# IN2-ViAUn/Exploration-of-Potential

Measured on AMD Instinct MI355X. Metric: training images/sec, YOLOX-l 24p 640x640 bf16, higher is better.
Workload: dtype bf16; 1 GPU; YOLOX-l-24p (CSPDarknet53+PAFPN+24p head) train step, 640x640, batch 20/GPU, 10 GTs/img, SimOTA + 24-circle GIoU loss, SGD nesterov; global_batch=20, parallelism=dp1, hip_graph=forward and backward as two lanes of captured segments, loss, update

## Files before the change

### exploration-of-potential_amd/csrc/elementwise.hip

```cpp
#include <stdio.h>
#include <stdlib.h>
#include "common.h"

namespace {

constexpr int MAX_BLOCKS = 2048;

__device__ __forceinline__ void load8(const bf16* p, float (&v)[8]) {
    bf16x8 t = *reinterpret_cast<const bf16x8*>(p);
#pragma unroll
    for (int i = 0; i < 8; ++i) v[i] = (float)t[i];
}
__device__ __forceinline__ void store8(bf16* p, const float (&v)[8]) {
    bf16x8 t;
#pragma unroll
    for (int i = 0; i < 8; ++i) t[i] = (bf16)v[i];
    *reinterpret_cast<bf16x8*>(p) = t;
}

struct RowMap {
    int tpr, rpb;
    __device__ RowMap(int C, int nt = 256) { tpr = C >> 3; rpb = tpr >= nt ? 1 : nt / tpr; }
};

template <int ACT, bool RES>
__global__ __launch_bounds__(256) void bn_act_fwd_kernel(const bf16* z, long ld_z, const long long* stats, int reps,
                                                         const float* gamma, const float* beta, float* rmean,
                                                         float* rvar, long* nbt, long* nbt2, float* save, bf16* y, long ld_y,
                                                         const bf16* res_, long ld_res, long M, int C, float eps,
                                                         float momentum) {
    constexpr int act = ACT;
    const bf16* res = RES ? res_ : nullptr;
    extern __shared__ float lds[];
    const int CP = C + (C >> 3);
    float* sc = lds;
    float* sh = lds + CP;
    auto pad = [](int c) { return c + (c >> 3); };
    for (int c = threadIdx.x; c < C; c += 256) {
        long long i1 = 0, i2 = 0;
        const float gmm = gamma[c], bta = beta[c];
        for (int rb = 0; rb < reps; rb += 8) {
            long long a[8], b[8];
#pragma unroll
            for (int r = 0; r < 8; ++r) {
                const int rr = rb + r < reps ? rb + r : rb;
                a[r] = stats[(long)rr * 2 * C + c];
                b[r] = stats[(long)rr * 2 * C + C + c];
            }
#pragma unroll
            for (int r = 0; r < 8; ++r) {
                i1 += rb + r < reps ? a[r] : 0ll;
                i2 += rb + r < reps ? b[r] : 0ll;
            }
        }
        const float mean = from_fix(i1) / (float)M;
        float var = from_fix(i2) / (float)M - mean * mean;
        var = var < 0.f ? 0.f : var;
        const float invstd = rsqrtf(var + eps);
        const float s_ = gmm * invstd;
        sc[pad(c)] = s_;
        sh[pad(c)] = bta - mean * s_;
        if (blockIdx.x == 0) {
            save[c] = mean;
            save[C + c] = invstd;
            if (rmean) {
                const float unb = M > 1 ? var * (float)M / (float)(M - 1) : var;
                rmean[c] = (1.f - momentum) * rmean[c] + momentum * mean;
                rvar[c] = (1.f - momentum) * rvar[c] + momentum * unb;
            }
        }
    }
    if (blockIdx.x == 0 && threadIdx.x == 0) {
        if (nbt) *nbt += 1;
        if (nbt2) *nbt2 += 1;
    }
    __syncthreads();
    const int cgs = C >> 3;
    const long total = M * cgs;
    const long stride = (long)gridDim.x * 256;
    constexpr int U = 4;
    const bool fixed_group = stride % cgs == 0;
    const int g_fixed = (int)(((long)blockIdx.x * 256 + threadIdx.x) % cgs);
    float rsc[8], rsh[8];
#pragma unroll
    for (int j = 0; j < 8; ++j) { rsc[j] = sc[g_fixed * 9 + j]; rsh[j] = sh[g_fixed * 9 + j]; }
    const long m_fixed = ((long)blockIdx.x * 256 + threadIdx.x) / cgs, m_step = stride / cgs;
    int it = 0;
    for (long i = (long)blockIdx.x * 256 + threadIdx.x; i < total; i += U * stride, ++it) {
        long mm[U];
        int gg[U];
        bf16x8 v[U], r[U];
#pragma unroll
        for (int k = 0; k < U; ++k) {
            const long ik = i + k * stride;
            const bool ok = ik < total;
            if (fixed_group) {
                mm[k] = ok ? m_fixed + (long)(it * U + k) * m_step : -1;
                gg[k] = g_fixed;
            } else {
                mm[k] = ok ? ik / cgs : -1;
                gg[k] = ok ? (int)(ik - mm[k] * cgs) : 0;
            }
            if (ok) {
                v[k] = *reinterpret_cast<const bf16x8*>(z + mm[k] * ld_z + gg[k] * 8);
                if constexpr (RES) r[k] = *reinterpret_cast<const bf16x8*>(res + mm[k] * ld_res + gg[k] * 8);
            }
        }
#pragma unroll
        for (int k = 0; k < U; ++k) {
            if (mm[k] < 0) break;
            bf16x8 o;
#pragma unroll
            for (int j = 0; j < 8; ++j) {
                const float a_ = fixed_group ? rsc[j] : sc[gg[k] * 9 + j];
                const float b_ = fixed_group ? rsh[j] : sh[gg[k] * 9 + j];
                const float u = fmaf((float)v[k][j], a_, b_);
                if constexpr (RES) o[j] = (bf16)(act_fwd(u, act) + (float)r[k][j]);
                else o[j] = (bf16)act_fwd(u, act);
            }
            *reinterpret_cast<bf16x8*>(y + mm[k] * ld_y + gg[k] * 8) = o;
        }
    }
}


template <int UNROLL, int NT, int ACT>
__device__ __forceinline__ void bn_bwd_reduce_body(const bf16* dy, long ld_dy, const bf16* z, long ld_z,
                                                   const float* save, const float* gamma,
                                                   const float* beta, long long* dgamma, long long* dbeta,
                                                   long M, int C, int reps, const int bid, const int nblk) {
    constexpr int act = ACT;
    __shared__ float red[NT][8 + 1];
    const RowMap rm(C, NT);
    const int tid = threadIdx.x;
    for (int cg0 = 0; cg0 < (C >> 3); cg0 += NT) {
        const int cg = cg0 + tid % rm.tpr;
        const int slot = rm.tpr >= NT ? 0 : tid / rm.tpr;
        const bool active = slot < rm.rpb && cg < (C >> 3);
        float sg[8] = {0, 0, 0, 0, 0, 0, 0, 0}, sb[8] = {0, 0, 0, 0, 0, 0, 0, 0};
        if (active) {
            const long step = (long)nblk * rm.rpb;
            const long m_first = (long)bid * rm.rpb + slot;
            bf16x8 vdy[UNROLL], vz[UNROLL];
#pragma unroll
            for (int k = 0; k < UNROLL; ++k) {
                const long mm = m_first + k * step < M ? m_first + k * step : (m_first < M ? m_first : 0);
                vdy[k] = *reinterpret_cast<const bf16x8*>(dy + mm * ld_dy + cg * 8);
                vz[k] = *reinterpret_cast<const bf16x8*>(z + mm * ld_z + cg * 8);
            }
            __builtin_amdgcn_sched_barrier(0);
            float sc[8], sh[8], iv[8], mi[8];
#pragma unroll
            for (int j = 0; j < 8; ++j) {
                const int c = cg * 8 + j;
                const float mean = save[c], inv = save[C + c];
                sc[j] = gamma[c] * inv; sh[j] = beta[c] - mean * sc[j]; iv[j] = inv; mi[j] = mean * inv;
            }
            for (long m = m_first; m < M; m += UNROLL * step) {
#pragma unroll
                for (int k = 0; k < UNROLL; ++k) {
                    if (m + k * step >= M) break;
#pragma unroll
                    for (int j = 0; j < 8; ++j) {
                        const float zz = (float)vz[k][j];
                        const float du = (float)vdy[k][j] * act_grad(fmaf(zz, sc[j], sh[j]), act);
                        sb[j] += du;
                        sg[j] = fmaf(du, fmaf(zz, iv[j], -mi[j]), sg[j]);
                    }
                }
                if (m + UNROLL * step < M) {
#pragma unroll
                    for (int k = 0; k < UNROLL; ++k) {
                        const long mn = m + (UNROLL + k) * step;
                        const long mm = mn < M ? mn : m;
                        vdy[k] = *reinterpret_cast<const bf16x8*>(dy + mm * ld_dy + cg * 8);
                        vz[k] = *reinterpret_cast<const bf16x8*>(z + mm * ld_z + cg * 8);
                    }
                }
            }
        }
        const int ngrp = min(min(rm.tpr, NT), (C >> 3) - cg0);
#pragma unroll
        for (int half = 0; half < 2; ++half) {
#pragma unroll
            for (int j = 0; j < 8; ++j) red[tid][j] = half ? sb[j] : sg[j];
            __syncthreads();
            for (int t = tid; t < ngrp * 8; t += NT) {
                const int g = t >> 3, v = t & 7;
                float a = 0.f;
                for (int sl = 0; sl < rm.rpb; ++sl) a += red[sl * rm.tpr + g][v];
                long long* dst = (half ? dbeta : dgamma) + (long)(bid % reps) * 2 * C + (cg0 + g) * 8 + v;
                atomicAdd((unsigned long long*)dst, (unsigned long long)to_fix_g(a));
            }
            __syncthreads();
        }
    }
}

template <int UNROLL, int NT, int ACT>
__global__ __launch_bounds__(NT) void bn_act_bwd_reduce_kernel(const bf16* dy, long ld_dy, const bf16* z, long ld_z,
                                                               const float* save, const float* gamma,
                                                               const float* beta, long long* dgamma, long long* dbeta,
                                                               long M, int C, int reps) {
    bn_bwd_reduce_body<UNROLL, NT, ACT>(dy, ld_dy, z, ld_z, save, gamma, beta, dgamma, dbeta, M, C, reps, (int)blockIdx.x, (int)gridDim.x);
}

template <int UNROLL, int ACT, bool ACC, bool COH>
__device__ __forceinline__ void bn_bwd_apply_body(const bf16* dy, long ld_dy, const bf16* z, long ld_z,
                                                  const float* save, const float* gamma, const float* beta,
                                                  const long long* dgamma, const long long* dbeta, float* ggrad,
                                                  float* bgrad, bf16* dz, long ld_dz, long M, int C, int reps, const int bid, const int nblk) {
    constexpr int act = ACT;
    const RowMap rm(C);
    const int tid = threadIdx.x;
    const float invM = 1.f / (float)M;
    extern __shared__ float folded[];
    for (int i = tid; i < 2 * C; i += 256) {
        const long long* src = i < C ? dgamma + i : dbeta + (i - C);
        long long acc = 0;
        bool bad = false;
        for (int rb = 0; rb < reps; rb += 8) {
            long long a[8];
#pragma unroll
            for (int r = 0; r < 8; ++r) {
                const long long* q = src + (long)(rb + r < reps ? rb + r : rb) * 2 * C;
                a[r] = COH ? __hip_atomic_load(q, __ATOMIC_RELAXED, __HIP_MEMORY_SCOPE_AGENT) : *q;
            }
#pragma unroll
            for (int r = 0; r < 8; ++r) {
                acc += rb + r < reps ? a[r] : 0ll;
                bad = bad || fixg_bad(a[r]);
            }
        }
        folded[i] = bad ? __builtin_nanf("") : from_fix_g(acc);
    }
    __syncthreads();
    for (int cg = tid % rm.tpr; cg < (C >> 3); cg += 256) {
        const int slot = rm.tpr >= 256 ? 0 : tid / rm.tpr;
        if (slot >= rm.rpb) break;
        float sc[8], sh[8], k1[8], k2[8], k3[8];
        float cm[8], ci[8], cg_[8], cb[8], csg[8], csb[8];
        {
            const f32x4* pm = reinterpret_cast<const f32x4*>(save + cg * 8);
            const f32x4* pi = reinterpret_cast<const f32x4*>(save + C + cg * 8);
            const f32x4* pg = reinterpret_cast<const f32x4*>(gamma + cg * 8);
            const f32x4* pb = reinterpret_cast<const f32x4*>(beta + cg * 8);
            const f32x4 m0 = pm[0], m1 = pm[1], i0 = pi[0], i1 = pi[1], g0 = pg[0], g1 = pg[1], b0 = pb[0], b1 = pb[1];
            const f32x4 s0 = *reinterpret_cast<const f32x4*>(folded + cg * 8), s1 = *reinterpret_cast<const f32x4*>(folded + cg * 8 + 4);
            const f32x4 t0 = *reinterpret_cast<const f32x4*>(folded + C + cg * 8), t1 = *reinterpret_cast<const f32x4*>(folded + C + cg * 8 + 4);
#pragma unroll
            for (int j = 0; j < 4; ++j) {
                cm[j] = m0[j]; cm[4 + j] = m1[j]; ci[j] = i0[j]; ci[4 + j] = i1[j]; cg_[j] = g0[j]; cg_[4 + j] = g1[j]; cb[j] = b0[j]; cb[4 + j] = b1[j];
                csg[j] = s0[j]; csg[4 + j] = s1[j]; csb[j] = t0[j]; csb[4 + j] = t1[j];
            }
        }
#pragma unroll
        for (int j = 0; j < 8; ++j) {
            const float mean = cm[j], inv = ci[j], g = cg_[j];
            const float sg_ = csg[j], sb_ = csb[j];
            sc[j] = g * inv; sh[j] = cb[j] - mean * sc[j];
            k1[j] = g * inv;
            k3[j] = k1[j] * inv * (sg_ * invM);
            k2[j] = k1[j] * (sb_ * invM) - k3[j] * mean;
        }
        if (bid == 0 && slot == 0 && ggrad) {
            f32x4* pgg = reinterpret_cast<f32x4*>(ggrad + cg * 8);
            f32x4* pbg = reinterpret_cast<f32x4*>(bgrad + cg * 8);
            f32x4 a0 = pgg[0], a1 = pgg[1], c0 = pbg[0], c1 = pbg[1];
#pragma unroll
            for (int j = 0; j < 4; ++j) {
                a0[j] += csg[j]; a1[j] += csg[4 + j];
                c0[j] += csb[j]; c1[j] += csb[4 + j];
            }
            pgg[0] = a0; pgg[1] = a1; pbg[0] = c0; pbg[1] = c1;
        }
        const long step = (long)nblk * rm.rpb;
        for (long m = (long)bid * rm.rpb + slot; m < M; m += UNROLL * step) {
            bf16x8 vdy[UNROLL], vz[UNROLL];
#pragma unroll
            for (int k = 0; k < UNROLL; ++k) {
                const long mm = m + k * step;
                if (mm < M) {
                    vdy[k] = __builtin_nontemporal_load(reinterpret_cast<const bf16x8*>(dy + mm * ld_dy + cg * 8));
                    vz[k] = __builtin_nontemporal_load(reinterpret_cast<const bf16x8*>(z + mm * ld_z + cg * 8));
                }
            }
#pragma unroll
            for (int k = 0; k < UNROLL; ++k) {
                const long mm = m + k * step;
                if (mm >= M) break;
                bf16x8 o;
#pragma unroll
                for (int j = 0; j < 8; ++j) {
                    const float zz = (float)vz[k][j];
                    const float du = (float)vdy[k][j] * act_grad(fmaf(zz, sc[j], sh[j]), act);
                    o[j] = (bf16)fmaf(-k3[j], zz, fmaf(k1[j], du, -k2[j]));
                }
                if (ACC) {
                    const bf16x8 old = *reinterpret_cast<const bf16x8*>(dz + mm * ld_dz + cg * 8);
#pragma unroll
                    for (int j = 0; j < 8; ++j) o[j] = (bf16)((float)old[j] + (float)o[j]);
                }
                *reinterpret_cast<bf16x8*>(dz + mm * ld_dz + cg * 8) = o;
            }
        }
    }
}

template <int UNROLL, int ACT, bool ACC = false>
__global__ __launch_bounds__(256) void bn_act_bwd_apply_kernel(const bf16* dy, long ld_dy, const bf16* z, long ld_z,
                                                               const float* save, const float* gamma, const float* beta,
                                                               const long long* dgamma, const long long* dbeta, float* ggrad,
                                                               float* bgrad, bf16* dz, long ld_dz, long M, int C, int reps) {
    bn_bwd_apply_body<UNROLL, ACT, ACC, false>(dy, ld_dy, z, ld_z, save, gamma, beta, dgamma, dbeta, ggrad, bgrad, dz, ld_dz, M, C, reps,
                                               (int)blockIdx.x, (int)gridDim.x);
}

__device__ unsigned g_bn_barrier_timeouts;

template <int ACT>
__global__ __launch_bounds__(256) void bn_act_bwd_fused_kernel(const bf16* dy, long ld_dy, const bf16* z, long ld_z,
                                                               const float* save, const float* gamma, const float* beta,
                                                               long long* dgamma, long long* dbeta, float* ggrad, float* bgrad,
                                                               bf16* dz, long ld_dz, long M, int C, int reps, unsigned* bar) {
    const int bid = (int)blockIdx.x, nblk = (int)gridDim.x;
    bn_bwd_reduce_body<4, 256, ACT>(dy, ld_dy, z, ld_z, save, gamma, beta, dgamma, dbeta, M, C, reps, bid, nblk);
    __syncthreads();
    if (threadIdx.x == 0) {
        __threadfence();
        __hip_atomic_fetch_add(bar, 1u, __ATOMIC_RELEASE, __HIP_MEMORY_SCOPE_AGENT);
        int tries = 0;
        while (__hip_atomic_load(bar, __ATOMIC_ACQUIRE, __HIP_MEMORY_SCOPE_AGENT) < (unsigned)nblk) {
            __builtin_amdgcn_s_sleep(2);
            if (++tries > (1 << 16)) { atomicAdd(&g_bn_barrier_timeouts, 1u); break; }
        }
    }
    __syncthreads();
    bn_bwd_apply_body<4, ACT, false, true>(dy, ld_dy, z, ld_z, save, gamma, beta, dgamma, dbeta, ggrad, bgrad, dz, ld_dz, M, C, reps, bid, nblk);
}

int flat_grid(long M, int C, int per_thread) {
    long blocks = (M * (C >> 3) + 256L * per_thread - 1) / (256L * per_thread);
    return (int)(blocks < 1 ? 1 : (blocks > MAX_BLOCKS ? MAX_BLOCKS : blocks));
}
int rows_grid(long M, int C, int rows_per_thread, int max_blocks, int nt = 256) {
    int tpr = C >> 3;
    int rpb = tpr >= nt ? 1 : nt / tpr;
    long blocks = (M + (long)rpb * rows_per_thread - 1) / ((long)rpb * rows_per_thread);
    return (int)(blocks < 1 ? 1 : (blocks > max_blocks ? max_blocks : blocks));
}

__global__ __launch_bounds__(256) void stem_pack_kernel(const float* img, bf16* rows, int B, int IH, int IW, int ld) {
    constexpr int TP = 32;
    __shared__ __attribute__((aligned(16))) bf16 tile[TP][120];
    const int FH = IH >> 1, FW = IW >> 1;
    const long npix = (long)B * FH * FW;
    const int chunks = ld >> 3;
    for (long p0 = (long)blockIdx.x * TP; p0 < npix; p0 += (long)gridDim.x * TP) {
        for (int it = threadIdx.x; it < 9 * TP; it += 256) {
            const int tap = it / TP, lp = it - tap * TP;
            const long pix = p0 + lp;
            float v[12] = {0.f, 0.f, 0.f, 0.f, 0.f, 0.f, 0.f, 0.f, 0.f, 0.f, 0.f, 0.f};
            if (pix < npix) {
                const int n = (int)(pix / ((long)FH * FW));
                const int rem = (int)(pix - (long)n * FH * FW);
                const int oy = rem / FW, ox = rem - oy * FW;
                const int fy = oy + tap / 3 - 1, fx = ox + tap % 3 - 1;
                if (fy >= 0 && fy < FH && fx >= 0 && fx < FW) {
#pragma unroll
                    for (int ch = 0; ch < 3; ++ch)
#pragma unroll
                        for (int yp = 0; yp < 2; ++yp) {
                            const float2 t = *reinterpret_cast<const float2*>(img + (((long)n * 3 + ch) * IH + 2 * fy + yp) * IW + 2 * fx);
                            v[(0 * 2 + yp) * 3 + ch] = t.x;
                            v[(1 * 2 + yp) * 3 + ch] = t.y;
                        }
                }
            }
#pragma unroll
            for (int j = 0; j < 12; ++j) tile[lp][tap * 12 + j] = (bf16)v[j];
        }
        if (threadIdx.x < TP) {
#pragma unroll
            for (int j = 108; j < 120; ++j) tile[threadIdx.x][j] = (bf16)0.f;
        }
        __syncthreads();
        for (int it = threadIdx.x; it < TP * chunks; it += 256) {
            const int lp = it / chunks, c = it - lp * chunks;
            const long pix = p0 + lp;
            if (pix >= npix) continue;
            bf16x8 o = {0, 0, 0, 0, 0, 0, 0, 0};
            if (c * 8 < 120) o = *reinterpret_cast<const bf16x8*>(&tile[lp][c * 8]);
            *reinterpret_cast<bf16x8*>(rows + pix * ld + c * 8) = o;
        }
        __syncthreads();
    }
}

__global__ __launch_bounds__(256) void focus_pack_kernel(const float* img, bf16* out, int B, int IH, int IW) {
    const int FH = IH >> 1, FW = IW >> 1;
    const long npix = (long)B * FH * FW;
    for (long pix = (long)blockIdx.x * 256 + threadIdx.x; pix < npix; pix += (long)gridDim.x * 256) {
        const int n = (int)(pix / ((long)FH * FW));
        const int rem = (int)(pix - (long)n * FH * FW);
        const int fy = rem / FW, fx = rem - fy * FW;
        float v[12];
#pragma unroll
        for (int ch = 0; ch < 3; ++ch)
#pragma unroll
            for (int yp = 0; yp < 2; ++yp) {
                const float2 t = *reinterpret_cast<const float2*>(img + (((long)n * 3 + ch) * IH + 2 * fy + yp) * IW + 2 * fx);
                v[(0 * 2 + yp) * 3 + ch] = t.x;
                v[(1 * 2 + yp) * 3 + ch] = t.y;
            }
        bf16x8 lo, hi = {0, 0, 0, 0, 0, 0, 0, 0};
#pragma unroll
        for (int j = 0; j < 8; ++j) lo[j] = (bf16)v[j];
#pragma unroll
        for (int j = 8; j < 12; ++j) hi[j - 8] = (bf16)v[j];
        *reinterpret_cast<bf16x8*>(out + pix * 16) = lo;
        *reinterpret_cast<bf16x8*>(out + pix * 16 + 8) = hi;
    }
}

__global__ __launch_bounds__(256) void spp_fwd_kernel(const bf16* x, long ld_x, bf16* y5, bf16* y9, bf16* y13, long ld_y,
                                                      uint8_t* idx, int B, int H, int W, int C) {
    const int cgs = C >> 3;
    const long total = (long)B * H * W * cgs;
    const long plane = (long)B * H * W * C;
    for (long i = (long)blockIdx.x * 256 + threadIdx.x; i < total; i += (long)gridDim.x * 256) {
        const int cg = (int)(i % cgs);
        const long pix = i / cgs;
        const int n = (int)(pix / (H * W));
        const int rem = (int)(pix - (long)n * H * W);
        const int py = rem / W, px = rem - py * W;
        float m5[8], m9[8], m13[8];
        uint8_t i5[8], i9[8], i13[8];
#pragma unroll
        for (int j = 0; j < 8; ++j) { m5[j] = m9[j] = m13[j] = -INFINITY; i5[j] = i9[j] = i13[j] = 0x88; }
        for (int dy = -6; dy <= 6; ++dy) {
            const int yy = py + dy;
            if (yy < 0 || yy >= H) continue;
            for (int dx = -6; dx <= 6; ++dx) {
                const int xx = px + dx;
                if (xx < 0 || xx >= W) continue;
                float v[8];
                load8(x + ((long)(n * H + yy) * W + xx) * ld_x + cg * 8, v);
                const uint8_t code = (uint8_t)(((dy + 8) << 4) | (dx + 8));
                const bool in9 = dy >= -4 && dy <= 4 && dx >= -4 && dx <= 4;
                const bool in5 = dy >= -2 && dy <= 2 && dx >= -2 && dx <= 2;
#pragma unroll
                for (int j = 0; j < 8; ++j) {
                    if (v[j] > m13[j] || v[j] != v[j]) { m13[j] = v[j]; i13[j] = code; }
                    if (in9 && (v[j] > m9[j] || v[j] != v[j])) { m9[j] = v[j]; i9[j] = code; }
                    if (in5 && (v[j] > m5[j] || v[j] != v[j])) { m5[j] = v[j]; i5[j] = code; }
                }
            }
        }
        store8(y5 + pix * ld_y + cg * 8, m5);
        store8(y9 + pix * ld_y + cg * 8, m9);
        store8(y13 + pix * ld_y + cg * 8, m13);
        uint8_t* ip = idx + pix * C + cg * 8;
#pragma unroll
        for (int j = 0; j < 8; ++j) { ip[j] = i5[j]; ip[plane + j] = i9[j]; ip[2 * plane + j] = i13[j]; }
    }
}

__global__ __launch_bounds__(256) void spp_row_kernel(const bf16* x, long ld_x, bf16* h, uint8_t* hx, int B, int H, int W, int C) {
    const int cgs = C >> 3;
    const long total = (long)B * H * W * cgs;
    const long plane = (long)B * H * W * C;
    for (long i = (long)blockIdx.x * 256 + threadIdx.x; i < total; i += (long)gridDim.x * 256) {
        const int cg = (int)(i % cgs);
        const long pix = i / cgs;
// ... 541 lines not shown
constexpr int WF_NONE = -2147483647 - 1;
__global__ __launch_bounds__(256) void sgd_kernel(float* p, const float* g, float* buf, long n, float lr, float mom,
                                                  float gscale, const int* first_flag, const float* hp, float* ema,
                                                  long base = 0, const int* wf_delta = nullptr, bf16* wf = nullptr) {
    const int first = *first_flag;
    float d = 0.f, omd = 0.f;
    if (hp) { lr = hp[0]; mom = hp[1]; gscale = hp[2]; d = hp[3]; omd = hp[4]; }
    for (long i = ((long)blockIdx.x * 256 + threadIdx.x) * 4; i < n; i += (long)gridDim.x * 1024) {
        if (i + 3 < n) {
            f32x4 gv = *reinterpret_cast<const f32x4*>(g + i);
            f32x4 pv = *reinterpret_cast<const f32x4*>(p + i);
            f32x4 bv = first ? (f32x4){0.f, 0.f, 0.f, 0.f} : *reinterpret_cast<const f32x4*>(buf + i);
            const int wd = wf_delta ? wf_delta[(base + i) >> 6] : WF_NONE;
#pragma unroll
            for (int j = 0; j < 4; ++j) {
                const float gg = gv[j] * gscale;
                bv[j] = first ? gg : mom * bv[j] + gg;
                pv[j] -= lr * (gg + mom * bv[j]);
            }
            *reinterpret_cast<f32x4*>(buf + i) = bv;
            *reinterpret_cast<f32x4*>(p + i) = pv;
            if (wd != WF_NONE) {
                bf16x4 o;
#pragma unroll
                for (int j = 0; j < 4; ++j) o[j] = (bf16)pv[j];
                *reinterpret_cast<bf16x4*>(wf + (base + i + wd)) = o;
            }
            if (ema) {
                f32x4 ev = *reinterpret_cast<const f32x4*>(ema + i);
#pragma unroll
                for (int j = 0; j < 4; ++j) ev[j] = ema_step(ev[j], pv[j], d, omd);
                *reinterpret_cast<f32x4*>(ema + i) = ev;
            }
        } else {
            for (long k = i; k < n; ++k) {
                const float gg = g[k] * gscale;
                const float b = first ? gg : mom * buf[k] + gg;
                buf[k] = b;
                p[k] -= lr * (gg + mom * b);
                if (ema) ema[k] = ema_step(ema[k], p[k], d, omd);
                const int wd = wf_delta ? wf_delta[(base + k) >> 6] : WF_NONE;
                if (wd != WF_NONE) wf[base + k + wd] = (bf16)p[k];
            }
        }
    }
}

__global__ __launch_bounds__(256) void ema_kernel(float* ema, const float* src, long n, float d, float omd, const float* hp) {
    if (hp) { d = hp[3]; omd = hp[4]; }
    for (long i = (long)blockIdx.x * 256 + threadIdx.x; i < n; i += (long)gridDim.x * 256) ema[i] = ema_step(ema[i], src[i], d, omd);
}

__global__ void set_hparams_kernel(float* hp, float lr, float mom, float gscale, float d, float omd) {
    hp[0] = lr; hp[1] = mom; hp[2] = gscale; hp[3] = d; hp[4] = omd;
}
__global__ void clear_flag_kernel(int* f) { *f = 0; }

int cap_grid(long work_items) {
    long b = (work_items + 255) / 256;
    return (int)(b < 1 ? 1 : (b > MAX_BLOCKS ? MAX_BLOCKS : b));
}

}

#define S_ (hipStream_t) stream

extern "C" int ep24_bn_act_fwd(const void* z, int64_t ld_z, const int64_t* stats, int reps, const float* gamma,
                               const float* beta, float* running_mean, float* running_var, int64_t* num_batches,
                               int64_t* num_batches2, float* save, void* y, int64_t ld_y, const void* residual, int64_t ld_res,
                               int64_t M, int C, float eps, float momentum, int act, void* stream) {
    EP24_REQUIRE(act >= 0 && act <= 3, EP24_E_ARG, "bn_act_fwd: act=%d is none of 0 identity, 1 SiLU, 2 ReLU, 3 LeakyReLU(0.1)", act);
    EP24_REQUIRE(z && stats && gamma && beta && save && y, EP24_E_ARG, "bn_act_fwd: null pointer");
    EP24_REQUIRE(C % 8 == 0 && ld_z % 8 == 0 && ld_y % 8 == 0 && (!residual || ld_res % 8 == 0), EP24_E_ARG,
                 "bn_act_fwd: C=%d / strides must be multiples of 8", C);
    EP24_REQUIRE(M > 0 && reps > 0, EP24_E_ARG, "bn_act_fwd: empty");
    const int fw_per = (C >= 1024 || (C <= 128 && M * C >= (12L << 20))) ? 8 : 4;
    auto kfn = residual ? (act == 1 ? bn_act_fwd_kernel<1, true> : act == 2 ? bn_act_fwd_kernel<2, true> : act == 3 ? bn_act_fwd_kernel<3, true> : bn_act_fwd_kernel<0, true>)
                        : (act == 1 ? bn_act_fwd_kernel<1, false> : act == 2 ? bn_act_fwd_kernel<2, false> : act == 3 ? bn_act_fwd_kernel<3, false> : bn_act_fwd_kernel<0, false>);
    hipLaunchKernelGGL(kfn, dim3(flat_grid(M, C, fw_per)), dim3(256), 2 * (C + C / 8) * sizeof(float), S_, (const bf16*)z, ld_z, (const long long*)stats, reps, gamma,
                       beta, running_mean, running_var, (long*)num_batches, (long*)num_batches2, save, (bf16*)y, ld_y, (const bf16*)residual,
                       ld_res, M, C, eps, momentum);
    EP24_LAUNCH_CHECK("ep24_bn_act_fwd");
    return EP24_OK;
}

extern "C" int ep24_bn_act_bwd_reduce(const void* dy, int64_t ld_dy, const void* z, int64_t ld_z, const float* save,
                                      const float* gamma, const float* beta, int64_t* dgamma, int64_t* dbeta, int64_t M, int C,
                                      int act, int reps, void* stream) {
    EP24_REQUIRE(act >= 0 && act <= 3, EP24_E_ARG, "bn_act_bwd_reduce: act=%d is none of 0 identity, 1 SiLU, 2 ReLU, 3 LeakyReLU(0.1)", act);
    EP24_REQUIRE(dy && z && save && gamma && beta && dgamma && dbeta && reps > 0, EP24_E_ARG, "bn_act_bwd_reduce: null pointer / reps");
    EP24_REQUIRE(C % 8 == 0 && ld_dy % 8 == 0 && ld_z % 8 == 0, EP24_E_ARG, "bn_act_bwd_reduce: alignment");
    int red_cap = 512;
    int red_rows = 4;
    auto kfn = act == 1 ? bn_act_bwd_reduce_kernel<4, 256, 1> : act == 2 ? bn_act_bwd_reduce_kernel<4, 256, 2> : act == 3 ? bn_act_bwd_reduce_kernel<4, 256, 3> : bn_act_bwd_reduce_kernel<4, 256, 0>;
    hipLaunchKernelGGL(kfn, dim3(rows_grid(M, C, red_rows, red_cap, 256)), dim3(256), 0, S_, (const bf16*)dy, ld_dy, (const bf16*)z, ld_z,
                       save, gamma, beta, (long long*)dgamma, (long long*)dbeta, M, C, reps);
    EP24_LAUNCH_CHECK("ep24_bn_act_bwd_reduce");
    return EP24_OK;
}

extern "C" int ep24_bn_act_bwd_apply(const void* dy, int64_t ld_dy, const void* z, int64_t ld_z, const float* save,
                                     const float* gamma, const float* beta, const int64_t* dgamma, const int64_t* dbeta,
                                     float* gamma_grad, float* beta_grad, void* dz, int64_t ld_dz, int64_t M, int C, int act,
                                     int reps, void* stream) {
    EP24_REQUIRE(act >= 0 && act <= 3, EP24_E_ARG, "bn_act_bwd_apply: act=%d is none of 0 identity, 1 SiLU, 2 ReLU, 3 LeakyReLU(0.1)", act);
    EP24_REQUIRE(dy && z && save && gamma && beta && dgamma && dbeta && dz && reps > 0, EP24_E_ARG, "bn_act_bwd_apply: null pointer / reps");
    EP24_REQUIRE(C % 8 == 0 && ld_dy % 8 == 0 && ld_z % 8 == 0 && ld_dz % 8 == 0, EP24_E_ARG, "bn_act_bwd_apply: alignment");
    EP24_REQUIRE((((uintptr_t)save | (uintptr_t)gamma | (uintptr_t)beta) & 15) == 0, EP24_E_ARG,
                 "bn_act_bwd_apply: save / gamma / beta must be 16-byte aligned (they are read as vectors)");
    EP24_REQUIRE((((uintptr_t)gamma_grad | (uintptr_t)beta_grad) & 15) == 0, EP24_E_ARG, "bn_act_bwd_apply: gamma_grad / beta_grad must be 16-byte aligned");
    const int ap_rows = M * C <= (16L << 20) ? 8 : 16, ap_cap = 2048;
    auto kfn = act == 1 ? bn_act_bwd_apply_kernel<4, 1> : act == 2 ? bn_act_bwd_apply_kernel<4, 2> : act == 3 ? bn_act_bwd_apply_kernel<4, 3> : bn_act_bwd_apply_kernel<4, 0>;
    hipLaunchKernelGGL(kfn, dim3(rows_grid(M, C, ap_rows, ap_cap)), dim3(256), 2 * (size_t)C * sizeof(float), S_, (const bf16*)dy, ld_dy,
                       (const bf16*)z, ld_z, save, gamma, beta, (const long long*)dgamma, (const long long*)dbeta, gamma_grad, beta_grad,
                       (bf16*)dz, ld_dz, M, C, reps);
    EP24_LAUNCH_CHECK("ep24_bn_act_bwd_apply");
    return EP24_OK;
}

extern "C" int ep24_bn_act_bwd_fused(const void* dy, int64_t ld_dy, const void* z, int64_t ld_z, const float* save, const float* gamma,
                                     const float* beta, int64_t* dgamma, int64_t* dbeta, float* gamma_grad, float* beta_grad, void* dz,
                                     int64_t ld_dz, int64_t M, int C, int act, int reps, int32_t* barrier, void* stream) {
    EP24_REQUIRE(act >= 0 && act <= 3, EP24_E_ARG, "bn_act_bwd_fused: act=%d is none of 0 identity, 1 SiLU, 2 ReLU, 3 LeakyReLU(0.1)", act);
    EP24_REQUIRE(dy && z && save && gamma && beta && dgamma && dbeta && dz && barrier && reps > 0, EP24_E_ARG, "bn_act_bwd_fused: null pointer / reps");
    EP24_REQUIRE(C % 8 == 0 && C <= 2048 && ld_dy % 8 == 0 && ld_z % 8 == 0 && ld_dz % 8 == 0, EP24_E_ARG, "bn_act_bwd_fused: alignment / C <= 2048");
    EP24_REQUIRE((((uintptr_t)save | (uintptr_t)gamma | (uintptr_t)beta | (uintptr_t)gamma_grad | (uintptr_t)beta_grad) & 15) == 0, EP24_E_ARG,
                 "bn_act_bwd_fused: save / gamma / beta and their gradients must be 16-byte aligned (they are read as vectors)");
    int grid = rows_grid(M, C, 4, 256, 256);
    auto kfn = act == 1 ? bn_act_bwd_fused_kernel<1> : act == 2 ? bn_act_bwd_fused_kernel<2> : act == 3 ? bn_act_bwd_fused_kernel<3> : bn_act_bwd_fused_kernel<0>;
    hipLaunchKernelGGL(kfn, dim3(grid), dim3(256), 2 * (size_t)C * sizeof(float), S_, (const bf16*)dy, ld_dy, (const bf16*)z, ld_z, save, gamma, beta,
                       (long long*)dgamma, (long long*)dbeta, gamma_grad, beta_grad, (bf16*)dz, ld_dz, M, C, reps, (unsigned*)barrier);
    EP24_LAUNCH_CHECK("ep24_bn_act_bwd_fused");
    return EP24_OK;
}

namespace ep24_igemm {
int bn_barrier_timeouts() {
    unsigned v = 0;
    if (hipMemcpyFromSymbol(&v, HIP_SYMBOL(g_bn_barrier_timeouts), sizeof(v)) != hipSuccess) return -1;
    return (int)v;
}
}

extern "C" int ep24_bn_act_bwd_apply_acc(const void* dy, int64_t ld_dy, const void* z, int64_t ld_z, const float* save,
                                         const float* gamma, const float* beta, const int64_t* dgamma, const int64_t* dbeta,
                                         float* gamma_grad, float* beta_grad, void* dz, int64_t ld_dz, int64_t M, int C, int act,
                                         int reps, void* stream) {
    EP24_REQUIRE(act >= 0 && act <= 3, EP24_E_ARG, "bn_act_bwd_apply_acc: act=%d is none of 0 identity, 1 SiLU, 2 ReLU, 3 LeakyReLU(0.1)", act);
    EP24_REQUIRE(dy && z && save && gamma && beta && dgamma && dbeta && dz && reps > 0, EP24_E_ARG, "bn_act_bwd_apply_acc: null pointer / reps");
    EP24_REQUIRE(C % 8 == 0 && ld_dy % 8 == 0 && ld_z % 8 == 0 && ld_dz % 8 == 0, EP24_E_ARG, "bn_act_bwd_apply_acc: alignment");
    EP24_REQUIRE((((uintptr_t)save | (uintptr_t)gamma | (uintptr_t)beta) & 15) == 0, EP24_E_ARG,
                 "bn_act_bwd_apply_acc: save / gamma / beta must be 16-byte aligned (they are read as vectors)");
    EP24_REQUIRE((((uintptr_t)gamma_grad | (uintptr_t)beta_grad) & 15) == 0, EP24_E_ARG, "bn_act_bwd_apply_acc: gamma_grad / beta_grad must be 16-byte aligned");
    auto kfn = act == 1 ? bn_act_bwd_apply_kernel<4, 1, true> : act == 2 ? bn_act_bwd_apply_kernel<4, 2, true> : act == 3 ? bn_act_bwd_apply_kernel<4, 3, true> : bn_act_bwd_apply_kernel<4, 0, true>;
    hipLaunchKernelGGL(kfn, dim3(rows_grid(M, C, 16, 2048)), dim3(256), 2 * (size_t)C * sizeof(float), S_, (const bf16*)dy, ld_dy, (const bf16*)z, ld_z, save, gamma, beta,
                       (const long long*)dgamma, (const long long*)dbeta, gamma_grad, beta_grad, (bf16*)dz, ld_dz, M, C, reps);
    EP24_LAUNCH_CHECK("ep24_bn_act_bwd_apply_acc");
    return EP24_OK;
}

extern "C" int ep24_stem_pack(const float* images, void* rows, int64_t ld, int B, int H, int W, void* stream) {
    EP24_REQUIRE(images && rows && H % 2 == 0 && W % 2 == 0 && B > 0 && ld >= 108 && ld % 8 == 0, EP24_E_ARG, "stem_pack: bad arguments");
    long sp_blocks = ((long)B * (H / 2) * (W / 2) + 31) / 32;
    hipLaunchKernelGGL(stem_pack_kernel, dim3((unsigned)(sp_blocks > 16384 ? 16384 : sp_blocks)), dim3(256), 0, S_, images,
                       (bf16*)rows, B, H, W, (int)ld);
    EP24_LAUNCH_CHECK("ep24_stem_pack");
    return EP24_OK;
}

extern "C" int ep24_focus_pack(const float* images, void* f16, int B, int H, int W, void* stream) {
    EP24_REQUIRE(images && f16 && H % 2 == 0 && W % 2 == 0 && B > 0 && (reinterpret_cast<unsigned long long>(images) & 7) == 0, EP24_E_ARG,
                 "focus_pack: bad arguments");
    const long blocks = ((long)B * (H / 2) * (W / 2) + 255) / 256;
    hipLaunchKernelGGL(focus_pack_kernel, dim3((unsigned)(blocks > 65536 ? 65536 : blocks)), dim3(256), 0, S_, images, (bf16*)f16, B, H, W);
    EP24_LAUNCH_CHECK("ep24_focus_pack");
    return EP24_OK;
}

extern "C" int ep24_spp_fwd(const void* x, int64_t ld_x, void* y5, void* y9, void* y13, int64_t ld_y, uint8_t* idx, int B,
                            int H, int W, int C, void* scratch, void* stream) {
    EP24_REQUIRE(x && y5 && y9 && y13 && idx && C % 8 == 0 && ld_x % 8 == 0 && ld_y % 8 == 0, EP24_E_ARG, "spp_fwd: bad arguments");
    if (scratch) {
        const long n = (long)B * H * W * C;
        bf16* h = (bf16*)scratch;
        uint8_t* hx = (uint8_t*)scratch + 6 * n;
        hipLaunchKernelGGL(spp_row_kernel, dim3(cap_grid(n / 8)), dim3(256), 0, S_, (const bf16*)x, ld_x, h, hx, B, H, W, C);
        hipLaunchKernelGGL(spp_col_kernel, dim3(cap_grid(n / 8)), dim3(256), 0, S_, (const bf16*)h, (const uint8_t*)hx, (bf16*)y5,
                           (bf16*)y9, (bf16*)y13, ld_y, idx, B, H, W, C);
        EP24_LAUNCH_CHECK("ep24_spp_fwd");
        return EP24_OK;
    }
    hipLaunchKernelGGL(spp_fwd_kernel, dim3(cap_grid((long)B * H * W * (C / 8))), dim3(256), 0, S_, (const bf16*)x, ld_x,
                       (bf16*)y5, (bf16*)y9, (bf16*)y13, ld_y, idx, B, H, W, C);
    EP24_LAUNCH_CHECK("ep24_spp_fwd");
    return EP24_OK;
}

extern "C" int ep24_spp_bwd(const void* dy5, const void* dy9, const void* dy13, int64_t ld_dy, const uint8_t* idx, void* dx,
                            int64_t ld_dx, int accumulate, int B, int H, int W, int C, void* stream) {
    EP24_REQUIRE(dy5 && dy9 && dy13 && idx && dx && C % 8 == 0 && ld_dy % 8 == 0 && ld_dx % 8 == 0, EP24_E_ARG, "spp_bwd: bad arguments");
    const size_t lds = (size_t)H * W * 112;
    if (lds <= 64 * 1024 && H * W <= 1024)
        hipLaunchKernelGGL(spp_bwd_lds_kernel, dim3(C / 8, B), dim3(256), lds, S_, (const bf16*)dy5, (const bf16*)dy9, (const bf16*)dy13,
                           ld_dy, idx, (bf16*)dx, ld_dx, accumulate, B, H, W, C);
    else
        hipLaunchKernelGGL(spp_bwd_kernel, dim3(cap_grid((long)B * H * W * (C / 8))), dim3(256), 0, S_, (const bf16*)dy5,
                           (const bf16*)dy9, (const bf16*)dy13, ld_dy, idx, (bf16*)dx, ld_dx, accumulate, B, H, W, C);
    EP24_LAUNCH_CHECK("ep24_spp_bwd");
    return EP24_OK;
}

extern "C" int ep24_upsample2_fwd(const void* x, int64_t ld_x, void* y, int64_t ld_y, int B, int H, int W, int C, void* stream) {
    EP24_REQUIRE(x && y && C % 8 == 0 && ld_x % 8 == 0 && ld_y % 8 == 0, EP24_E_ARG, "upsample2_fwd: bad arguments");
    hipLaunchKernelGGL(upsample2_fwd_kernel, dim3(cap_grid((long)B * 4 * H * W * (C / 8))), dim3(256), 0, S_, (const bf16*)x,
                       ld_x, (bf16*)y, ld_y, B, H, W, C);
    EP24_LAUNCH_CHECK("ep24_upsample2_fwd");
    return EP24_OK;
}

extern "C" int ep24_upsample2_bwd(const void* dy, int64_t ld_dy, void* dx, int64_t ld_dx, int accumulate, int B, int H, int W,
                                  int C, void* stream) {
    EP24_REQUIRE(dy && dx && C % 8 == 0 && ld_dy % 8 == 0 && ld_dx % 8 == 0, EP24_E_ARG, "upsample2_bwd: bad arguments");
    hipLaunchKernelGGL(upsample2_bwd_kernel, dim3(cap_grid((long)B * H * W * (C / 8))), dim3(256), 0, S_, (const bf16*)dy, ld_dy,
                       (bf16*)dx, ld_dx, accumulate, B, H, W, C);
    EP24_LAUNCH_CHECK("ep24_upsample2_bwd");
    return EP24_OK;
}

extern "C" int ep24_rows_copy(const void* src, int64_t ld_src, void* dst, int64_t ld_dst, int accumulate, int64_t M, int C,
                              void* stream) {
    EP24_REQUIRE(src && dst && C % 8 == 0 && ld_src % 8 == 0 && ld_dst % 8 == 0, EP24_E_ARG, "rows_copy: bad arguments");
    hipLaunchKernelGGL(rows_copy_kernel, dim3(cap_grid(M * (C / 8))), dim3(256), 0, S_, (const bf16*)src, ld_src, (bf16*)dst,
                       ld_dst, accumulate, M, C);
    EP24_LAUNCH_CHECK("ep24_rows_copy");
    return EP24_OK;
}

extern "C" int ep24_cast_f32_bf16(const float* src, void* dst, int64_t n, void* stream) {
    EP24_REQUIRE(src && dst && n % 4 == 0 && n >= 0, EP24_E_ARG, "cast_f32_bf16: n must be a multiple of 4");
    EP24_REQUIRE((uintptr_t)src % 16 == 0 && (uintptr_t)dst % 8 == 0, EP24_E_ARG, "cast_f32_bf16: src must be 16-byte, dst 8-byte aligned");
    if (n) hipLaunchKernelGGL(cast_f32_bf16_kernel, dim3(cap_grid(n / 4)), dim3(256), 0, S_, src, (bf16*)dst, (long)(n / 4));
    EP24_LAUNCH_CHECK("ep24_cast_f32_bf16");
    return EP24_OK;
}

extern "C" int ep24_cast_bf16_f32(const void* src, float* dst, int64_t n, void* stream) {
    EP24_REQUIRE(src && dst && n % 4 == 0 && n >= 0, EP24_E_ARG, "cast_bf16_f32: n must be a multiple of 4");
    EP24_REQUIRE((uintptr_t)src % 8 == 0 && (uintptr_t)dst % 16 == 0, EP24_E_ARG, "cast_bf16_f32: src must be 8-byte, dst 16-byte aligned");
    if (n) hipLaunchKernelGGL(cast_bf16_f32_kernel, dim3(cap_grid(n / 4)), dim3(256), 0, S_, (const bf16*)src, dst, (long)(n / 4));
    EP24_LAUNCH_CHECK("ep24_cast_bf16_f32");
    return EP24_OK;
}

extern "C" int ep24_head_decode_fwd(float* out, int B, int A, int a0, int H, int W, float stride, int ncols, float* origin,
                                    void* stream) {
    EP24_REQUIRE(out && a0 >= 0 && a0 + H * W <= A && ncols >= 27, EP24_E_ARG, "head_decode_fwd: bad arguments");
    hipLaunchKernelGGL(decode_fwd_kernel, dim3(cap_grid((long)B * H * W * 26)), dim3(256), 0, S_, out, B, A, a0, H, W, stride, ncols, origin);
    EP24_LAUNCH_CHECK("ep24_head_decode_fwd");
    return EP24_OK;
}

extern "C" int ep24_head_decode_bwd(const float* dout, const float* out, void* d_regobj, void* d_cls, int B, int A, int a0,
                                    int H, int W, float stride, int ncols, const float* d_origin, void* stream) {
    EP24_REQUIRE(dout && out && d_regobj && d_cls && a0 >= 0 && a0 + H * W <= A && ncols > 27, EP24_E_ARG,
                 "head_decode_bwd: bad arguments");
    hipLaunchKernelGGL(decode_bwd_kernel, dim3(cap_grid((long)B * H * W * (4 + (ncols - 27 + 7) / 8))), dim3(256), 0, S_, dout, out, (bf16*)d_regobj,
                       (bf16*)d_cls, B, A, a0, H, W, stride, ncols, d_origin);
    EP24_LAUNCH_CHECK("ep24_head_decode_bwd");
    return EP24_OK;
}

extern "C" int ep24_colsum_splits(int64_t M) {
    long blocks = (M + 3) / 4;
    return (int)(blocks > 64 ? 64 : (blocks < 1 ? 1 : blocks));
}

extern "C" int ep24_colsum_slab(const void* g, int64_t ld, float* slab, int64_t M, int N, void* stream) {
    EP24_REQUIRE(g && slab && N > 0 && N <= 2048 && M > 0 && ld % 8 == 0 && ld >= ((N + 7) / 8) * 8, EP24_E_ARG,
                 "colsum_slab: bad arguments (rows must be padded to a multiple of 8 columns)");
    hipLaunchKernelGGL(colsum_slab_kernel, dim3((unsigned)ep24_colsum_splits(M)), dim3(256), 0, S_, (const bf16*)g, ld, slab, M, N);
    EP24_LAUNCH_CHECK("ep24_colsum_slab");
    return EP24_OK;
}

extern "C" int ep24_colsum(const void* g, int64_t ld, float* db, int64_t M, int N, void* stream) {
    EP24_REQUIRE(g && db && N > 0, EP24_E_ARG, "colsum: bad arguments");
    long blocks = (M + 3) / 4;
    if (blocks > 512) blocks = 512;
    hipLaunchKernelGGL(colsum_kernel, dim3((unsigned)blocks), dim3(256), 0, S_, (const bf16*)g, ld, db, M, N);
    EP24_LAUNCH_CHECK("ep24_colsum");
    return EP24_OK;
}

extern "C" int ep24_pack_weights(const float* w, int64_t ld_w, void* w_fwd, void* w_dgrad, int Cout, int T, int Cin, int Cin_pad,
                                 int Cout_pad, void* stream) {
    EP24_REQUIRE(w && (w_fwd || w_dgrad) && Cin_pad >= Cin && Cout_pad >= Cout, EP24_E_ARG, "pack_weights: bad arguments");
    long n = (long)Cout * T * Cin;
    hipLaunchKernelGGL(pack_weights_kernel, dim3(cap_grid(n)), dim3(256), 0, S_, w, ld_w, (bf16*)w_fwd, (bf16*)w_dgrad, Cout, T, Cin,
                       Cin_pad, Cout_pad);
    EP24_LAUNCH_CHECK("ep24_pack_weights");
    return EP24_OK;
}

extern "C" int ep24_sgd_nesterov(float* p, const float* g, float* buf, int64_t n, float lr, float momentum, float grad_scale,
                                 int32_t* first_flag, void* stream) {
    EP24_REQUIRE(p && g && buf && first_flag && n > 0, EP24_E_ARG, "sgd_nesterov: bad arguments");
    EP24_REQUIRE(((uintptr_t)p | (uintptr_t)g | (uintptr_t)buf) % 16 == 0, EP24_E_ARG, "sgd_nesterov: 16-byte alignment");
// ... 102 lines not shown
```

Baseline: 1041 images/s.

## Prefetch BN backward apply loads ahead of the stat fold and pipeline rows

The BN+activation backward apply body now issues the first row loads (dy, z, old dz) and the per-channel constants before folding the fixed-point gamma/beta partials. This hides global-load latency behind the reduction and the barrier. The row loop becomes software-pipelined: each iteration computes from registers and immediately prefetches the next rows, with the next channel group's loads requested early. The kernels also get a 4-waves-per-EU occupancy hint, and the accumulate variant drops from unroll 4 to 2 to save registers. The risks are extra register pressure and redundant clamped loads for non-owner threads.

```diff
diff --git a/exploration-of-potential_amd/csrc/elementwise.hip b/exploration-of-potential_amd/csrc/elementwise.hip
--- a/exploration-of-potential_amd/csrc/elementwise.hip
+++ b/exploration-of-potential_amd/csrc/elementwise.hip
@@ -17,6 +17,8 @@
     for (int i = 0; i < 8; ++i) t[i] = (bf16)v[i];
     *reinterpret_cast<bf16x8*>(p) = t;
 }
+
+#define BN_4_WAVES __attribute__((amdgpu_waves_per_eu(4)))
 
 struct RowMap {
     int tpr, rpb;
@@ -215,100 +217,128 @@
     const int tid = threadIdx.x;
     const float invM = 1.f / (float)M;
     extern __shared__ float folded[];
-    for (int i = tid; i < 2 * C; i += 256) {
-        const long long* src = i < C ? dgamma + i : dbeta + (i - C);
-        long long acc = 0;
-        bool bad = false;
+    const int slot = rm.tpr >= 256 ? 0 : tid / rm.tpr;
+    const bool owner = slot < rm.rpb;
+    const long step = (long)nblk * rm.rpb;
+    const long m_first = (long)bid * rm.rpb + slot;
+    const long m_own = owner && m_first < M ? m_first : 0;
+    bf16x8 dyA[UNROLL], zA[UNROLL], oldA[UNROLL];
+    auto request = [&](long m0, long alt, bool mine, int cg, bf16x8 (&vdy)[UNROLL], bf16x8 (&vz)[UNROLL], bf16x8 (&vold)[UNROLL]) __attribute__((always_inline)) {
+#pragma unroll
+        for (int k = 0; k < UNROLL; ++k) {
+            long mm = mine && m0 + k * step < M ? m0 + k * step : alt;
+            asm volatile("" : "+v"(mm));
+            vdy[k] = __builtin_nontemporal_load(reinterpret_cast<const bf16x8*>(dy + mm * ld_dy + cg * 8));
+            vz[k] = __builtin_nontemporal_load(reinterpret_cast<const bf16x8*>(z + mm * ld_z + cg * 8));
+            if constexpr (ACC) vold[k] = *reinterpret_cast<const bf16x8*>(dz + mm * ld_dz + cg * 8);
+        }
+    };
+    f32x4 cv[8], gv[4];
+    const bool publish = bid == 0 && slot == 0 && ggrad;
+    auto request_consts = [&](int cg) __attribute__((always_inline)) {
+        const f32x4* pm = reinterpret_cast<const f32x4*>(save + cg * 8);
+        const f32x4* pi = reinterpret_cast<const f32x4*>(save + C + cg * 8);
+        const f32x4* pg = reinterpret_cast<const f32x4*>(gamma + cg * 8);
+        const f32x4* pb = reinterpret_cast<const f32x4*>(beta + cg * 8);
+        cv[0] = pm[0]; cv[1] = pm[1]; cv[2] = pi[0]; cv[3] = pi[1]; cv[4] = pg[0]; cv[5] = pg[1]; cv[6] = pb[0]; cv[7] = pb[1];
+    };
+    auto request_grads = [&](int cg) __attribute__((always_inline)) {
+        const f32x4* pgg = reinterpret_cast<const f32x4*>((ggrad ? ggrad : gamma) + cg * 8);
+        const f32x4* pbg = reinterpret_cast<const f32x4*>((ggrad ? bgrad : beta) + cg * 8);
+        gv[0] = pgg[0]; gv[1] = pgg[1]; gv[2] = pbg[0]; gv[3] = pbg[1];
+    };
+    const int cg_first = tid % rm.tpr;
+    request_consts(cg_first);
+    request(m_first, m_own, owner, cg_first, dyA, zA, oldA);
+    __builtin_amdgcn_sched_barrier(0);
+    for (unsigned c = tid; c < (unsigned)C; c += 256) {
+        long long accg = 0, accb = 0;
+        bool badg = false, badb = false;
         for (int rb = 0; rb < reps; rb += 8) {
-            long long a[8];
+            long long a[8], b[8];
 #pragma unroll
             for (int r = 0; r < 8; ++r) {
-                const long long* q = src + (long)(rb + r < reps ? rb + r : rb) * 2 * C;
-                a[r] = COH ? __hip_atomic_load(q, __ATOMIC_RELAXED, __HIP_MEMORY_SCOPE_AGENT) : *q;
+                const long roff = (long)(rb + r < reps ? rb + r : rb) * 2 * C;
+                a[r] = COH ? __hip_atomic_load(dgamma + roff + c, __ATOMIC_RELAXED, __HIP_MEMORY_SCOPE_AGENT) : (dgamma + roff)[c];
+                b[r] = COH ? __hip_atomic_load(dbeta + roff + c, __ATOMIC_RELAXED, __HIP_MEMORY_SCOPE_AGENT) : (dbeta + roff)[c];
             }
 #pragma unroll
             for (int r = 0; r < 8; ++r) {
-                acc += rb + r < reps ? a[r] : 0ll;
-                bad = bad || fixg_bad(a[r]);
-            }
-        }
-        folded[i] = bad ? __builtin_nanf("") : from_fix_g(acc);
-    }
+                accg += rb + r < reps ? a[r] : 0ll;
+                badg = badg || fixg_bad(a[r]);
+                accb += rb + r < reps ? b[r] : 0ll;
+                badb = badb || fixg_bad(b[r]);
+            }
+        }
+        folded[c] = badg ? __builtin_nanf("") : from_fix_g(accg);
+        folded[C + c] = badb ? __builtin_nanf("") : from_fix_g(accb);
+    }
+    request_grads(cg_first);
     __syncthreads();
-    for (int cg = tid % rm.tpr; cg < (C >> 3); cg += 256) {
-        const int slot = rm.tpr >= 256 ? 0 : tid / rm.tpr;
-        if (slot >= rm.rpb) break;
+    if (!owner) return;
+    for (int cg = cg_first; cg < (C >> 3); cg += 256) {
         float sc[8], sh[8], k1[8], k2[8], k3[8];
-        float cm[8], ci[8], cg_[8], cb[8], csg[8], csb[8];
-        {
-            const f32x4* pm = reinterpret_cast<const f32x4*>(save + cg * 8);
-            const f32x4* pi = reinterpret_cast<const f32x4*>(save + C + cg * 8);
-            const f32x4* pg = reinterpret_cast<const f32x4*>(gamma + cg * 8);
-            const f32x4* pb = reinterpret_cast<const f32x4*>(beta + cg * 8);
-            const f32x4 m0 = pm[0], m1 = pm[1], i0 = pi[0], i1 = pi[1], g0 = pg[0], g1 = pg[1], b0 = pb[0], b1 = pb[1];
-            const f32x4 s0 = *reinterpret_cast<const f32x4*>(folded + cg * 8), s1 = *reinterpret_cast<const f32x4*>(folded + cg * 8 + 4);
-            const f32x4 t0 = *reinterpret_cast<const f32x4*>(folded + C + cg * 8), t1 = *reinterpret_cast<const f32x4*>(folded + C + cg * 8 + 4);
-#pragma unroll
-            for (int j = 0; j < 4; ++j) {
-                cm[j] = m0[j]; cm[4 + j] = m1[j]; ci[j] = i0[j]; ci[4 + j] = i1[j]; cg_[j] = g0[j]; cg_[4 + j] = g1[j]; cb[j] = b0[j]; cb[4 + j] = b1[j];
-                csg[j] = s0[j]; csg[4 + j] = s1[j]; csb[j] = t0[j]; csb[4 + j] = t1[j];
-            }
-        }
-#pragma unroll
-        for (int j = 0; j < 8; ++j) {
-            const float mean = cm[j], inv = ci[j], g = cg_[j];
-            const float sg_ = csg[j], sb_ = csb[j];
-            sc[j] = g * inv; sh[j] = cb[j] - mean * sc[j];
-            k1[j] = g * inv;
-            k3[j] = k1[j] * inv * (sg_ * invM);
-            k2[j] = k1[j] * (sb_ * invM) - k3[j] * mean;
-        }
-        if (bid == 0 && slot == 0 && ggrad) {
-            f32x4* pgg = reinterpret_cast<f32x4*>(ggrad + cg * 8);
-            f32x4* pbg = reinterpret_cast<f32x4*>(bgrad + cg * 8);
-            f32x4 a0 = pgg[0], a1 = pgg[1], c0 = pbg[0], c1 = pbg[1];
-#pragma unroll
-            for (int j = 0; j < 4; ++j) {
-                a0[j] += csg[j]; a1[j] += csg[4 + j];
-                c0[j] += csb[j]; c1[j] += csb[4 + j];
-            }
-            pgg[0] = a0; pgg[1] = a1; pbg[0] = c0; pbg[1] = c1;
-        }
-        const long step = (long)nblk * rm.rpb;
-        for (long m = (long)bid * rm.rpb + slot; m < M; m += UNROLL * step) {
-            bf16x8 vdy[UNROLL], vz[UNROLL];
+#pragma unroll
+        for (int h = 0; h < 2; ++h) {
+            const f32x4 sgv = *reinterpret_cast<const f32x4*>(folded + cg * 8 + 4 * h);
+            const f32x4 sbv = *reinterpret_cast<const f32x4*>(folded + C + cg * 8 + 4 * h);
+#pragma unroll
+            for (int q = 0; q < 4; ++q) {
+                const int j = 4 * h + q;
+                const float mean = cv[h][q], inv = cv[2 + h][q], g = cv[4 + h][q];
+                const float sg_ = sgv[q], sb_ = sbv[q];
+                sc[j] = g * inv; sh[j] = cv[6 + h][q] - mean * sc[j];
+                k1[j] = g * inv;
+                k3[j] = k1[j] * inv * (sg_ * invM);
+                k2[j] = k1[j] * (sb_ * invM) - k3[j] * mean;
+            }
+            if (publish) {
+                f32x4 a0 = gv[h], c0 = gv[2 + h];
+#pragma unroll
+                for (int q = 0; q < 4; ++q) { a0[q] += sgv[q]; c0[q] += sbv[q]; }
+                reinterpret_cast<f32x4*>(ggrad + cg * 8)[h] = a0;
+                reinterpret_cast<f32x4*>(bgrad + cg * 8)[h] = c0;
+            }
+            __builtin_amdgcn_sched_barrier(0);
+        }
+        long ody = m_first * ld_dy + cg * 8, oz = m_first * ld_z + cg * 8, odz = m_first * ld_dz + cg * 8;
+        const long sdy = step * ld_dy, sz = step * ld_z, sdz = step * ld_dz;
+        for (long m = m_first; m < M; m += UNROLL * step, ody += UNROLL * sdy, oz += UNROLL * sz, odz += UNROLL * sdz) {
+            asm volatile("" : "+v"(ody), "+v"(oz), "+v"(odz));
 #pragma unroll
             for (int k = 0; k < UNROLL; ++k) {
-                const long mm = m + k * step;
-                if (mm < M) {
-                    vdy[k] = __builtin_nontemporal_load(reinterpret_cast<const bf16x8*>(dy + mm * ld_dy + cg * 8));
-                    vz[k] = __builtin_nontemporal_load(reinterpret_cast<const bf16x8*>(z + mm * ld_z + cg * 8));
-                }
-            }
-#pragma unroll
-            for (int k = 0; k < UNROLL; ++k) {
-                const long mm = m + k * step;
-                if (mm >= M) break;
+                if (m + k * step >= M) break;
                 bf16x8 o;
 #pragma unroll
                 for (int j = 0; j < 8; ++j) {
-                    const float zz = (float)vz[k][j];
-                    const float du = (float)vdy[k][j] * act_grad(fmaf(zz, sc[j], sh[j]), act);
+                    const float zz = (float)zA[k][j];
+                    const float du = (float)dyA[k][j] * act_grad(fmaf(zz, sc[j], sh[j]), act);
                     o[j] = (bf16)fmaf(-k3[j], zz, fmaf(k1[j], du, -k2[j]));
                 }
-                if (ACC) {
-                    const bf16x8 old = *reinterpret_cast<const bf16x8*>(dz + mm * ld_dz + cg * 8);
-#pragma unroll
-                    for (int j = 0; j < 8; ++j) o[j] = (bf16)((float)old[j] + (float)o[j]);
-                }
-                *reinterpret_cast<bf16x8*>(dz + mm * ld_dz + cg * 8) = o;
-            }
+                if constexpr (ACC) {
+#pragma unroll
+                    for (int j = 0; j < 8; ++j) o[j] = (bf16)((float)oldA[k][j] + (float)o[j]);
+                }
+                *reinterpret_cast<bf16x8*>(dz + odz + k * sdz) = o;
+                if (m + (UNROLL + k) * step < M) {
+                    dyA[k] = __builtin_nontemporal_load(reinterpret_cast<const bf16x8*>(dy + ody + (UNROLL + k) * sdy));
+                    zA[k] = __builtin_nontemporal_load(reinterpret_cast<const bf16x8*>(z + oz + (UNROLL + k) * sz));
+                    if constexpr (ACC) oldA[k] = *reinterpret_cast<const bf16x8*>(dz + odz + (UNROLL + k) * sdz);
+                }
+            }
+        }
+        if (cg + 256 < (C >> 3)) {
+            long mf = m_first, mo = m_own;
+            asm volatile("" : "+v"(mf), "+v"(mo));
+            request_consts(cg + 256);
+            request_grads(cg + 256);
+            request(mf, mo, true, cg + 256, dyA, zA, oldA);
         }
     }
 }
 
 template <int UNROLL, int ACT, bool ACC = false>
-__global__ __launch_bounds__(256) void bn_act_bwd_apply_kernel(const bf16* dy, long ld_dy, const bf16* z, long ld_z,
+__global__ __launch_bounds__(256) BN_4_WAVES void bn_act_bwd_apply_kernel(const bf16* dy, long ld_dy, const bf16* z, long ld_z,
                                                                const float* save, const float* gamma, const float* beta,
                                                                const long long* dgamma, const long long* dbeta, float* ggrad,
                                                                float* bgrad, bf16* dz, long ld_dz, long M, int C, int reps) {
@@ -319,7 +349,7 @@
 __device__ unsigned g_bn_barrier_timeouts;
 
 template <int ACT>
-__global__ __launch_bounds__(256) void bn_act_bwd_fused_kernel(const bf16* dy, long ld_dy, const bf16* z, long ld_z,
+__global__ __launch_bounds__(256) BN_4_WAVES void bn_act_bwd_fused_kernel(const bf16* dy, long ld_dy, const bf16* z, long ld_z,
                                                                const float* save, const float* gamma, const float* beta,
                                                                long long* dgamma, long long* dbeta, float* ggrad, float* bgrad,
                                                                bf16* dz, long ld_dz, long M, int C, int reps, unsigned* bar) {
@@ -1167,7 +1197,7 @@
     EP24_REQUIRE((((uintptr_t)save | (uintptr_t)gamma | (uintptr_t)beta) & 15) == 0, EP24_E_ARG,
                  "bn_act_bwd_apply_acc: save / gamma / beta must be 16-byte aligned (they are read as vectors)");
     EP24_REQUIRE((((uintptr_t)gamma_grad | (uintptr_t)beta_grad) & 15) == 0, EP24_E_ARG, "bn_act_bwd_apply_acc: gamma_grad / beta_grad must be 16-byte aligned");
-    auto kfn = act == 1 ? bn_act_bwd_apply_kernel<4, 1, true> : act == 2 ? bn_act_bwd_apply_kernel<4, 2, true> : act == 3 ? bn_act_bwd_apply_kernel<4, 3, true> : bn_act_bwd_apply_kernel<4, 0, true>;
+    auto kfn = act == 1 ? bn_act_bwd_apply_kernel<2, 1, true> : act == 2 ? bn_act_bwd_apply_kernel<2, 2, true> : act == 3 ? bn_act_bwd_apply_kernel<2, 3, true> : bn_act_bwd_apply_kernel<2, 0, true>;
     hipLaunchKernelGGL(kfn, dim3(rows_grid(M, C, 16, 2048)), dim3(256), 2 * (size_t)C * sizeof(float), S_, (const bf16*)dy, ld_dy, (const bf16*)z, ld_z, save, gamma, beta,
                        (const long long*)dgamma, (const long long*)dbeta, gamma_grad, beta_grad, (bf16*)dz, ld_dz, M, C, reps);
     EP24_LAUNCH_CHECK("ep24_bn_act_bwd_apply_acc");
```

Result: no change. 1042 images/s (median of 2 runs) (+0.1%).
